# zhangyi-3/UCDIR

Hardware: AMD Instinct MI355X
Metric: restored images/sec at 50-step p_sample_loop, 256x256 SID (higher is better)
Workload: dtype bf16

## Files before the change

### ucdir_amd/csrc/conv_sk.hip.h

```cpp
#pragma once
#include "asmops.hip.h"
#include "conv_halo.hip.h"
#include "akgm_ws.hip.h"

struct ConvSkP {
    const bf16_t* A; long long a_par_stride;
    const bf16_t* B0; const bf16_t* B1; int c0, ld0, ld1;
    int nchunks;
    int nb, H, W, Wp, Hp;
    int ns, Ws, Wpe, HpWpe, npos;
    float inv_per_b, inv_HpWpe, inv_Wpe;
    int ntiles, rowtiles, npar;
    int nhp;
    int nfeat;
    float alpha; int fold; int act;
    const stat_t* stats0; const stat_t* stats1; double inv_count;
    const float* bias; const float* Tb; const float* Tg; int tab_ld;
    const bf16_t* res; int res_ld;
    bf16_t* out; int out_ld;
    stat_t* stats_out;
    int units, ndp;
    float* partial;
    int alt_units; const bf16_t* alt_A; const float* alt_bias; bf16_t* alt_out; int alt_out_ld;
    int mix_wt, mix_nt, mix_nhp, mix_nunits, mix_nndp, mix_q0, mix_srt;
    unsigned long long* dbg;
};

template <int MW, int NW = 8>
struct CvSk {
    static constexpr int NWN = NW / MW;
    static constexpr int NPX = 64 * NWN;
    static constexpr int ROWS = 128 * MW;
    static constexpr int STAGE = 8192 * MW;
    static constexpr int PW = 8 * MW / NW;
    static constexpr bool LDS_TAB = NW == 8;
    static constexpr int OFF_W = 0;
    static constexpr int OFF_TB = 4 * STAGE;
    static constexpr int OFF_TG = OFF_TB + (LDS_TAB ? 9 * ROWS * 4 : 0);
    static constexpr int OFF_MS = OFF_TG + (LDS_TAB ? 9 * ROWS * 4 : 0);
    static constexpr int MAXB = 64;
    static constexpr int OFF_H = OFF_MS + MAXB * 8;
    static constexpr int THREADS = 64 * NW;
    static constexpr int NHW = NW == 4 ? 6 : (MW == 2 ? 4 : 7);
    static constexpr int NHP_MAX = NW * NHW;
    static constexpr int LDS_MAX = NW == 8 ? 160 * 1024 : 80 * 1024;
    __host__ __device__ static constexpr int lds_bytes(int nhp) { return OFF_H + 2 * nhp * 1024; }
    __host__ __device__ static constexpr int part_floats() { return ROWS * NPX; }
};

#ifdef UCDIR_TIMING
#define SK_STAMP() do { if (dbg_on && dbg_n < 120) p.dbg[dbg_off + dbg_n++] = __builtin_amdgcn_s_memtime(); } while (0)
#else
#define SK_STAMP() do {} while (0)
#endif

template <int N>
__device__ __forceinline__ void sk_wait_vm() { asm volatile("s_waitcnt vmcnt(%0)" :: "n"(N) : "memory"); }

struct SkSched {
    int units, ndp, nch, G;
    long long tc;
    __host__ __device__ SkSched(int units_, int ndp_, int nch_, int G_) : units(units_), ndp(ndp_), nch(nch_), G(G_), tc((long long)(units_ - ndp_) * nch_) {}
    __host__ __device__ long long start(int g) const { return tc * g / G; }
};

__device__ __forceinline__ int sk_udiv(int q, int d, float inv_d) {
    int t = (int)((float)q * inv_d);
    t = t * d > q ? t - 1 : t;
    t = (t + 1) * d <= q ? t + 1 : t;
    return t;
}
__device__ __forceinline__ void sk_decode(const ConvSkP& p, int q, int& b, int& yp, int& xs, int& xpm) {
    const int per_b = p.ns * p.HpWpe;
    b = sk_udiv(q, per_b, p.inv_per_b);
    int r = q - b * per_b;
    int strip = 0;
    if (p.ns > 1) { strip = sk_udiv(r, p.HpWpe, p.inv_HpWpe); r -= strip * p.HpWpe; }
    yp = sk_udiv(r, p.Wpe, p.inv_Wpe); xs = r - yp * p.Wpe;
    xpm = strip * p.Ws + xs;
}

__device__ __forceinline__ void lds_read8f_asm(f32x2_t& v, unsigned addr) {
    asm volatile("ds_read_b64 %0, %1" : "=v"(v) : "v"(addr));
}

__device__ __forceinline__ stat_t wave_sum_ll_dpp(stat_t v) {
    auto step = [&](auto ctrl, auto rmask) {
        constexpr int C = decltype(ctrl)::value, RM = decltype(rmask)::value;
// ... 247 lines not shown
        __builtin_amdgcn_sched_barrier(0);
    }
#pragma unroll
    for (int n = 0; n < 2; ++n) {
        const int q = q0 + wn * 64 + n * 32 + l31;
        int b, yp, xs, xp;
        sk_decode(p, q, b, yp, xs, xp);
        const bool valid = q < p.npos && yp >= 1 && yp <= p.H && xs >= 1 && xs <= p.Ws && xp <= p.W;
        const long long opos = ((long long)b * p.Hp + yp) * p.Wp + xp;
#pragma unroll
        for (int f = 0; f < 4; ++f) {
            const int fo = rt * L::ROWS + f * 32 + 16 * hh;
            if (!valid || fo >= p.nfeat) continue;
            float v[16];
#pragma unroll
            for (int g4 = 0; g4 < 4; ++g4) {
                f32x4_t bv = {0.f, 0.f, 0.f, 0.f};
                if (p.alt_bias) bv = *reinterpret_cast<const f32x4_t*>(p.alt_bias + fo + 4 * g4);
#pragma unroll
                for (int e = 0; e < 4; ++e) v[4 * g4 + e] = acc[f][n][4 * g4 + e] + bv[e];
            }
            bf16_t* op = p.alt_out + opos * p.alt_out_ld + fo;
            *reinterpret_cast<uint4*>(op) = pack8_bf16(v);
            *reinterpret_cast<uint4*>(op + 8) = pack8_bf16(v + 8);
        }
    }
}

template <int MW, int NW, int NTAPS, int NF = 4>
__device__ __forceinline__ void conv_sk_body(const ConvSkP& p, unsigned char* smem, const int lid, const int G, const int units_arg, const int ndp_arg,
                                             const int qbase, const int nhp) {
    using L = CvSk<MW, NW>;
    static_assert(NF == 4 || (NF == 2 && MW == 1 && NW == 4), "short units: four waves of 64 x 64");
    constexpr int PWN = L::PW * NF / 4;
    constexpr int RSUB = 4 / NF;
    constexpr int NWN = L::NWN;
    const int tid = threadIdx.x, lane = tid & 63, l31 = lane & 31, hh = lane >> 5;
    const int wave = __builtin_amdgcn_readfirstlane(tid >> 6);
    const int wm = wave / NWN, wn = wave % NWN;
#ifdef UCDIR_TIMING
    const bool dbg_on = p.dbg && (lid == G / 2 + 3 || lid == G - 3) && (lane == 0) && (wave == NW - 1);
    const int dbg_off = lid == G - 3 ? 128 : 0;
    int dbg_n = 0;
#endif
    SK_STAMP();
    const int Wp = p.Wpe, nch = p.nchunks;
    const int HB = nhp * 1024;
    constexpr int NHW = L::NHW;
    constexpr int TA = NTAPS - 3 > 1 ? NTAPS - 3 : 1;
    constexpr int HPER = (NHW + TA - 1) / TA;

    const unsigned a_lane = L::OFF_W + (NF == 4 ? (4 * wm) * 2048 : 0) + lane * 16;
    unsigned bx[NTAPS];
    auto set_bx = [&](int py, int pxp) {
#pragma unroll
        for (int t = 0; t < NTAPS; ++t) {
            int ky, kx;
            if (NTAPS == 9) { ky = t / 3; kx = t - 3 * ky; } else { ky = py + (t >> 1); kx = pxp + (t & 1); }
            const int hp = wn * 64 + l31 + ky * Wp + kx;
            bx[t] = L::OFF_H + (hp << 6) + (((hh ^ (hp >> 2)) & 3) << 4);
        }
    };
    if (NTAPS == 9) set_bx(0, 0);
    const int hpos0 = (lane >> 2) - Wp - 1;
    const unsigned hsw = (unsigned)(((lane & 3) ^ ((lane >> 4) & 3)) << 3);
    auto piece_of = [&](int j) { const int i = j * NW + wave; return i < nhp ? i : nhp - 1; };

    const SkSched sch(units_arg, ndp_arg, nch, G);
    const long long c_beg = sch.start(lid), c_end = sch.start(lid + 1);
    const int ndp_mine = lid < ndp_arg ? (ndp_arg - lid + G - 1) / G : 0;
    long long cpos = c_beg;
    int dpi = 0;
    struct Seg { int unit, cb, ce, par, rt, tile; bool first_sk, ok; };
    auto next_segment = [&]() {
        Seg s; s.ok = true; s.first_sk = false;
        if (dpi < ndp_mine) { s.unit = lid + dpi * G; s.cb = 0; s.ce = nch; ++dpi; }
        else if (cpos < c_end) {
            const long long u = cpos / nch;
            s.unit = ndp_arg + (int)u; s.cb = (int)(cpos - u * nch);
            const long long e = (u + 1) * nch < c_end ? (u + 1) * nch : c_end;
            s.ce = (int)(e - u * nch);
            s.first_sk = cpos == c_beg;
            cpos = e;
        } else { s.ok = false; s.unit = 0; s.cb = 0; s.ce = 0; }
        int u = s.unit;
        const int RT = NF == 4 ? p.rowtiles : p.mix_srt;
        const int per_par = RT * p.ntiles;
        s.par = 0;
        if (p.npar > 1) { s.par = u / per_par; u -= s.par * per_par; }
        s.tile = u / RT; s.rt = u - s.tile * RT;
        return s;
    };

    unsigned hq[NHW];
    int ld_cur = 0;
    const bf16_t* hsrc = nullptr;
    auto halo_chunk = [&](int c) {
        int ch = c * 32;
        const bool first = ch < p.c0;
        const int ld = first ? p.ld0 : p.ld1;
        hsrc = first ? p.B0 + ch : p.B1 + (ch - p.c0);
        if (ld != ld_cur) {
#pragma unroll
            for (int j = 0; j < NHW; ++j) hq[j] = ((((hq[j] >> 1) - hsw) / (unsigned)ld_cur) * (unsigned)ld + hsw) * 2u;
            ld_cur = ld;
        }
    };
    const unsigned char* a_seg = nullptr;
    const unsigned lane16 = (unsigned)lane * 16u;
    int seg_cb = 0;
    auto issue_halo = [&](int j, int buf) {
        dma16_sbase(hsrc, hq[j], (unsigned)(L::OFF_H + piece_of(j) * 1024 + buf * HB));
    };
    auto issue_stage = [&](int k, int slot) {
#pragma unroll
        for (int j = 0; j < PWN; ++j)
            dma16_sbase(a_seg + (long long)k * L::STAGE + j * 1024, lane16, (unsigned)(L::OFF_W + slot * L::STAGE + (wave * PWN + j) * 1024));
    };
    constexpr int NTP = 10;
    auto issue_table = [&](int rt, int i, int buf) {
        const int seg = 2 * i + (lane >> 5);
        const float* src = reinterpret_cast<const float*>(p.A);
        if (seg == 0 || seg > 18) { if (p.bias) src = p.bias + rt * L::ROWS; }
        else if (seg < 10) { if (p.fold) src = p.Tb + (long long)(seg - 1) * p.tab_ld + rt * L::ROWS; }
        else if (p.fold) src = p.Tg + (long long)(seg - 10) * p.tab_ld + rt * L::ROWS;
        __builtin_amdgcn_global_load_lds((const GLOBAL_AS void*)(src + (lane & 31) * 4), (LDS_AS void*)(smem + L::OFF_H + buf * HB + i * 1024), 16, 0, 0);
    };
    int hb0 = 0;
    auto prefetch = [&](const Seg& s) {
        if (NTAPS != 9) set_bx(s.par >> 1, s.par & 1);
        const int q0 = qbase + s.tile * L::NPX;
#pragma unroll
        for (int j = 0; j < NHW; ++j) {
            int q = q0 + hpos0 + 16 * piece_of(j);
            q = q < 0 ? 0 : (q >= p.npos ? (q - p.npos < p.npos ? q - p.npos : 0) : q);
            int b, yp, xs, xp;
            sk_decode(p, q, b, yp, xs, xp);
            xp = xp < p.Wp ? xp : p.Wp - 1;
            hq[j] = (unsigned)((b * p.Hp + yp) * p.Wp + xp);
        }
        ld_cur = s.cb * 32 < p.c0 ? p.ld0 : p.ld1;
#pragma unroll
        for (int j = 0; j < NHW; ++j) hq[j] = (hq[j] * (unsigned)ld_cur + hsw) * 2u;
        halo_chunk(s.cb);
        a_seg = reinterpret_cast<const unsigned char*>(p.A + (long long)s.par * p.a_par_stride + ((long long)(s.rt / RSUB) * nch * NTAPS) * (L::STAGE / 2) +
                                                       (s.rt % RSUB) * (L::STAGE / 2 / RSUB) + (wave * PWN) * 512);
        seg_cb = s.cb;
#pragma unroll
        for (int j = 0; j < NHW; ++j) issue_halo(j, hb0);
#pragma unroll
        for (int k = 0; k < 4; ++k) issue_stage(s.cb * NTAPS + k, k);
    };

    Seg cur = next_segment();
    if (!cur.ok) return;
    int rt_cur = cur.rt;
    prefetch(cur);
    auto sample_range = [&](const Seg& s) {
        const int per_b = p.ns * p.HpWpe;
        const int b0 = sk_udiv(qbase + s.tile * L::NPX, per_b, p.inv_per_b);
        int b1 = sk_udiv(qbase + s.tile * L::NPX + L::NPX - 1, per_b, p.inv_per_b) + 1; b1 = b1 < p.nb ? b1 : p.nb;
        if (b0 < b1) sk_sample_table(p, reinterpret_cast<float*>(smem + L::OFF_MS) + 2 * b0, b0, b1, wave, NW, lane);
    };
    if (L::LDS_TAB) {
        sk_sample_table(p, reinterpret_cast<float*>(smem + L::OFF_MS), 0, p.nb, wave, NW, lane);
        sk_row_table<MW, NW>(p, smem, cur.rt, tid);
    } else sample_range(cur);

#pragma unroll 1
    while (true) {
        const Seg nxt = next_segment();
        const int cb = cur.cb, ce = cur.ce;
        f32x16_t acc[NF][2];
#pragma unroll
        for (int f = 0; f < NF; ++f)
#pragma unroll
            for (int n = 0; n < 2; ++n)
#pragma unroll
                for (int e = 0; e < 16; ++e) acc[f][n][e] = 0.f;

        HC_WAIT(0);
        __builtin_amdgcn_sched_barrier(0);
        asm volatile("s_waitcnt lgkmcnt(0)\n\ts_barrier" ::: "memory");
        SK_STAMP();

        bf16x8_t fa[2][NF], fb[2][2];
        auto reads = [&](auto tc, auto jc, int h, unsigned boff) {
            constexpr int t = decltype(tc)::value, jj = decltype(jc)::value;
            const unsigned aa = a_lane + (unsigned)((h & 3) * L::STAGE);
            lds_read16_asm<0 * 2048 + jj * 1024>(fa[jj][0], aa);
            lds_read16_asm<1 * 2048 + jj * 1024>(fa[jj][1], aa);
            if constexpr (NF == 4) {
                lds_read16_asm<2 * 2048 + jj * 1024>(fa[jj][2], aa);
                lds_read16_asm<3 * 2048 + jj * 1024>(fa[jj][3], aa);
            }
            const unsigned b0 = (bx[t] + boff) ^ (jj << 5);
            lds_read16_asm<0>(fb[jj][0], b0);
            lds_read16_asm<2048>(fb[jj][1], b0);
        };
        __builtin_amdgcn_sched_barrier(0);
        unsigned bcur = hb0 ? (unsigned)HB : 0u;
        reads(std::integral_constant<int, 0>{}, std::integral_constant<int, 0>{}, 0, bcur);
        reads(std::integral_constant<int, 0>{}, std::integral_constant<int, 1>{}, 0, bcur);

        int h = 0;
        const bool want_tab = !L::LDS_TAB && cb == 0 && ce == nch;
#pragma unroll 1
        for (int c = cb; c < ce; ++c) {
            const unsigned bnext = bcur ? 0u : (unsigned)HB;
            const int cn = c + 1 < ce ? c + 1 : c;
            halo_chunk(cn);
            static_for<0, NTAPS>([&](auto tc) {
                constexpr int t = decltype(tc)::value;
                constexpr int tn = (t + 1) % NTAPS;
                constexpr int tm1 = (t + NTAPS - 1) % NTAPS;
                const unsigned boffn = tn == 0 ? bnext : bcur;
                const unsigned aan = a_lane + (unsigned)(((h + 1) & 3) * L::STAGE);
                auto unit = [&](auto jc, auto&& shadow) {
                    constexpr int jj = decltype(jc)::value;
                    const unsigned b0 = (bx[tn] + boffn) ^ (jj << 5);
#define SK_MF(f, n) acc[f][n] = __builtin_amdgcn_mfma_f32_32x32x16_bf16(fa[jj][f], fb[jj][n], acc[f][n], 0, 0, 0); __builtin_amdgcn_sched_barrier(0)
                    if constexpr (NF == 2) {
                        SK_MF(0, 0); shadow(std::integral_constant<int, 0>{}); __builtin_amdgcn_sched_barrier(0);
                        SK_MF(1, 0); lds_read16_asm<0>(fb[jj][0], b0); shadow(std::integral_constant<int, 1>{}); __builtin_amdgcn_sched_barrier(0);
                        SK_MF(0, 1); lds_read16_asm<0 * 2048 + jj * 1024>(fa[jj][0], aan); shadow(std::integral_constant<int, 2>{}); __builtin_amdgcn_sched_barrier(0);
                        SK_MF(1, 1); lds_read16_asm<1 * 2048 + jj * 1024>(fa[jj][1], aan); lds_read16_asm<2048>(fb[jj][1], b0); __builtin_amdgcn_sched_barrier(0);
                    } else {
                    SK_MF(0, 0); shadow(std::integral_constant<int, 0>{}); __builtin_amdgcn_sched_barrier(0);
                    SK_MF(1, 0); shadow(std::integral_constant<int, 1>{}); __builtin_amdgcn_sched_barrier(0);
                    SK_MF(2, 0); shadow(std::integral_constant<int, 2>{}); __builtin_amdgcn_sched_barrier(0);
#ifdef SK_ABL_NOREAD
                    SK_MF(3, 0); SK_MF(0, 1); SK_MF(1, 1); SK_MF(2, 1); SK_MF(3, 1); (void)b0; (void)aan;
#else
                    SK_MF(3, 0); lds_read16_asm<0>(fb[jj][0], b0); __builtin_amdgcn_sched_barrier(0);
                    SK_MF(0, 1); lds_read16_asm<0 * 2048 + jj * 1024>(fa[jj][0], aan); __builtin_amdgcn_sched_barrier(0);
                    SK_MF(1, 1); lds_read16_asm<1 * 2048 + jj * 1024>(fa[jj][1], aan); __builtin_amdgcn_sched_barrier(0);
                    SK_MF(2, 1); lds_read16_asm<2 * 2048 + jj * 1024>(fa[jj][2], aan); __builtin_amdgcn_sched_barrier(0);
                    SK_MF(3, 1); lds_read16_asm<3 * 2048 + jj * 1024>(fa[jj][3], aan); lds_read16_asm<2048>(fb[jj][1], b0); __builtin_amdgcn_sched_barrier(0);
#endif
                    }
#undef SK_MF
                };
#ifndef SK_ABL_NOREAD
                lgkm_wait_asm<NF + 2>();
#endif
                unit(std::integral_constant<int, 0>{}, [&](auto) {});
#ifndef SK_ABL_NOREAD
                lgkm_wait_asm<NF + 2>();
#endif
                {
                    constexpr int j0p = tm1 * HPER < NHW ? tm1 * HPER : NHW, j1p = (tm1 + 1) * HPER < NHW ? (tm1 + 1) * HPER : NHW;
                    constexpr int c1 = tm1 < TA ? j1p - j0p : 0;
#ifndef SK_ABL_NODMA
                    sk_wait_vm<PWN + c1>();
#endif
#ifndef SK_ABL_NOBAR
                    asm volatile("s_barrier" ::: "memory");
#endif
                }
                unit(std::integral_constant<int, 1>{}, [&](auto sc) {
                    constexpr int sidx = decltype(sc)::value;
                    constexpr int j0 = t < TA ? (t * HPER < NHW ? t * HPER : NHW) : 0, j1 = t < TA ? ((t + 1) * HPER < NHW ? (t + 1) * HPER : NHW) : 0;
                    constexpr int nh = j1 - j0;
                    constexpr int total = nh + PWN;
                    static_for<0, total>([&](auto qc) {
                        constexpr int q = decltype(qc)::value;
#ifdef SK_ABL_NODMA
                        constexpr int sh = 99;
#else
                        constexpr int sh = q * 3 / total;
#endif
                        if constexpr (sh == sidx) {
                            if constexpr (q < nh) {
                                constexpr int j = j0 + q;
                                if (want_tab && c + 1 == ce && j * NW + wave < NTP) issue_table(cur.rt / RSUB, j * NW + wave, bnext ? 1 : 0);
                                else issue_halo(j, bnext ? 1 : 0);
                            } else {
                                constexpr int j = q - nh;
                                dma16_sbase(a_seg + (long long)(cb * NTAPS + h + 4) * L::STAGE + j * 1024, lane16, (unsigned)(L::OFF_W + (h & 3) * L::STAGE + (wave * PWN + j) * 1024));
                            }
                        }
                    });
                });
                ++h;
            });
            bcur = bnext;
        }
        asm volatile("s_waitcnt vmcnt(0) lgkmcnt(0)" ::: "memory");
#pragma unroll
        for (int jj = 0; jj < 2; ++jj) {
#pragma unroll
            for (int f = 0; f < NF; ++f) asm volatile("" : "+v"(fa[jj][f]));
            asm volatile("" : "+v"(fb[jj][0]), "+v"(fb[jj][1]));
        }
        __builtin_amdgcn_sched_barrier(0);
        asm volatile("s_barrier" ::: "memory");
        SK_STAMP();
        const bool same_rt = nxt.ok && (nxt.rt == rt_cur || !L::LDS_TAB);
        const unsigned tab_base = (unsigned)L::OFF_H + bcur;
        hb0 = bcur ? 0 : 1;
        if (same_rt) prefetch(nxt);
        __builtin_amdgcn_sched_barrier(0);

        if (NF != 4 || (cb == 0 && ce == nch)) {
            sk_epilogue<MW, NW, L::LDS_TAB ? 1 : 2, true, NF>(p, smem, nullptr, acc, cur.par, cur.rt / RSUB, qbase + cur.tile * L::NPX, wm, wn, lane, tab_base, -1,
                                                             (cur.rt % RSUB) * (32 * NF));
        } else if constexpr (NF == 4) {
            float* pw = p.partial + ((long long)(2 * lid + (cur.first_sk ? 0 : 1))) * L::part_floats() + wave * (128 * 64) + lane * 4;
#pragma unroll
            for (int f = 0; f < 4; ++f)
#pragma unroll
                for (int n = 0; n < 2; ++n)
#pragma unroll
                    for (int g4 = 0; g4 < 4; ++g4)
                        *reinterpret_cast<float4*>(pw + ((f * 2 + n) * 4 + g4) * 256) =
                            make_float4(acc[f][n][4 * g4], acc[f][n][4 * g4 + 1], acc[f][n][4 * g4 + 2], acc[f][n][4 * g4 + 3]);
        }
        SK_STAMP();
        if (!nxt.ok) break;
        if (!same_rt) {
            __syncthreads();
            if (L::LDS_TAB) sk_row_table<MW, NW>(p, smem, nxt.rt, tid);
            rt_cur = nxt.rt;
            prefetch(nxt);
        }
        if (!L::LDS_TAB) { __syncthreads(); sample_range(nxt); }
        cur = nxt;
    }
#ifdef UCDIR_TIMING
    if (dbg_on) p.dbg[dbg_off ? 254 : 255] = dbg_n;
#endif
}

template <int MW, int NW, int NTAPS>
__global__ __launch_bounds__(64 * NW, 2) void conv_sk_kernel(const ConvSkP p) {
    extern __shared__ __attribute__((aligned(16))) unsigned char smem[];
    int lid, G;
    {
        int nblk = gridDim.x, bid = blockIdx.x;
        bool alt = false;
        if (MW == 1 && NW == 4 && p.alt_units) {
// ... 106 lines not shown
```

### ucdir_amd/csrc/engine.hip

```cpp
#include <hip/hip_runtime.h>

#include <algorithm>
#include <cmath>
#include <cstdio>
#include <cstring>
#include <map>
#include <mutex>
#include <set>
#include <array>
#include <atomic>
#include <memory>
#include <string>
#include <vector>

#include "../../include/ucdir_hip.h"
#include "cgemm.hip.h"
#include "conv_halo.hip.h"
#include "akgm_halo.hip.h"
#include "akgm_pre.hip.h"
#include "akgm_ws.hip.h"
#include "akgm_ws32.hip.h"
#include "akgm_ws64.hip.h"
#include "conv_ws.hip.h"
#include "conv_sk.hip.h"
// ... 10 lines not shown
    int rows_pad = 0, Kpad = 0, ntaps = 0, cin = 0, cout = 0, TM = 128; bool fold = false;
    bf16_t* Aup = nullptr; int Kup = 0;
    bf16_t* A10 = nullptr; float* bias_res = nullptr;
    bf16_t* Aws = nullptr;
    bf16_t* Aws128 = nullptr;
    bf16_t* Aqkv = nullptr;
    bf16_t* Atile = nullptr;
    bf16_t* Ask[2] = {nullptr, nullptr}; bf16_t* Ask_up[2] = {nullptr, nullptr};
    long long sk_up_stride[2] = {0, 0};
    bf16_t* Ask1x1 = nullptr;
};
struct AkgmW {
    bf16_t* A = nullptr; float* bias = nullptr; float* Tb = nullptr; float* Tg = nullptr;
    float* Tbb = nullptr;
    bf16_t* Apre = nullptr;
    bf16_t* Aws32 = nullptr;
    bf16_t* Aws64 = nullptr;
    int C = 0, cg = 0, Kpad = 0;
};

static int pick_tm(int cout) { return cout >= 128 ? 128 : 64; }

static ConvW upload_conv(DevPool& pool, const float* w, const float* bias, const float* gamma, const float* beta,
                         int cout, int cin, int ks) {
    ConvW W;
    W.TM = pick_tm(cout);
    PackedConv P = pack_conv(w, bias, gamma, beta, cout, cin, ks, W.TM);
    W.A = pool.upload(P.A); W.bias = pool.upload(P.bias);
    W.fold = gamma != nullptr;
    if (W.fold) { W.Tb = pool.upload(P.Tb); W.Tg = pool.upload(P.Tg); }
    W.rows_pad = P.rows_pad; W.Kpad = P.Kpad; W.ntaps = P.ntaps; W.cin = cin; W.cout = cout;
    if (ks == 3 && cin == 64 && cout == 64 && P.Kpad == 576) W.Aws = pool.upload(pack_conv_ws(P));
    if (ks == 3 && cin % 32 == 0 && P.Kpad == 9 * cin && P.rows_pad % W.TM == 0) W.Atile = pool.upload(pack_conv_tiled(P, W.TM));
    if (ks == 3 && cin % 32 == 0 && P.Kpad == 9 * cin && cout % 128 == 0) {
        W.Ask[0] = pool.upload(pack_conv_sk(P.A, 1, P.rows_pad, P.Kpad, cin, 9, 1));
        if (cout % 256 == 0) W.Ask[1] = pool.upload(pack_conv_sk(P.A, 1, P.rows_pad, P.Kpad, cin, 9, 2));
    }
    if (ks == 1 && cin % 32 == 0 && P.Kpad == cin && cout % 128 == 0 && gamma == nullptr) W.Ask1x1 = pool.upload(pack_conv_sk(P.A, 1, P.rows_pad, P.Kpad, cin, 1, 1));
    if (ks == 1 && cout == 3 * cin && gamma != nullptr && (cin == 256 || cin == 512) && P.Kpad == cin && P.rows_pad >= cout) W.Aqkv = pool.upload(pack_qkv_ws(P, cin));
    return W;
}
static void upload_upconv(DevPool& pool, ConvW& W, const float* w, const float* bias) {
    PackedConv P = pack_upconv(w, bias, W.cout, W.cin, W.TM);
    W.Aup = pool.upload(P.A); W.Kup = P.Kpad;
    for (int mw = 1; mw <= 2; ++mw)
        if (W.cin % 32 == 0 && W.cout % (128 * mw) == 0) {
            std::vector<bf16_t> img = pack_conv_sk(P.A, 4, P.rows_pad, P.Kpad, W.cin, 4, mw);
            W.sk_up_stride[mw - 1] = (long long)((img.size() - (size_t)4 * 4 * mw * 2 * 512) / 4);
            W.Ask_up[mw - 1] = pool.upload(img);
        }
}
static AkgmW upload_akgm(DevPool& pool, const float* wsp, const float* bsp, const float* gamma, const float* beta, int C) {
    PackedAkgm P = pack_akgm(wsp, bsp, gamma, beta, C, 0);
    AkgmW W;
    W.A = pool.upload(P.A); W.bias = pool.upload(P.bias); W.Tb = pool.upload(P.Tb); W.Tg = pool.upload(P.Tg);
    W.C = C; W.cg = P.cg; W.Kpad = P.Kpad;
    {
        std::vector<float> tbb(P.Tb.size());
        const size_t n = P.bias.size();
        for (size_t i = 0; i < tbb.size(); ++i) tbb[i] = P.bias[i % n] + P.Tb[i];
        W.Tbb = pool.upload(tbb);
    }
    if (P.cg == 8 || P.cg == 16) W.Apre = pool.upload(pack_akgm_pre(wsp, gamma, C));
    if (P.cg == 32) W.Aws32 = pool.upload(pack_akgm_ws32(wsp, gamma, C));
    if (P.cg == 64 && C == 512) W.Aws64 = pool.upload(pack_akgm_ws64(wsp, gamma, C));
    return W;
}

struct ProfEntry { int key; double flops, bytes; int dH, dW, dCin, dCout; hipEvent_t e0 = nullptr, e1 = nullptr; };
struct Profiler {
    bool on = false;
    std::vector<ProfEntry> entries;
    std::vector<hipEvent_t> pool; size_t used = 0;
    hipEvent_t get() {
        if (used == pool.size()) { hipEvent_t e; HIPC(hipEventCreate(&e)); pool.push_back(e); }
        return pool[used++];
    }
    ~Profiler() { for (auto e : pool) (void)hipEventDestroy(e); }
};
static Profiler g_prof;
// ... 448 lines not shown
    p.Hi = x0.H; p.Wi = x0.W; p.Wpi = x0.W + 2;
    p.p0 = p.Wp + 1; p.pn = (y.H - 1) * p.Wp + y.W;
    p.ntaps = w.ntaps; p.cg = cin; p.cpt = cin / 8; p.cpt_shift = 0;
    p.nk = w.Kpad / CG_BK;
    p.tiles = (p.pn + CG_TP - 1) / CG_TP;
    p.rowtiles = w.rows_pad / w.TM;
    p.nbatch = y.B;
    p.fold = w.fold ? 1 : 0; p.act = c.act;
    if (w.fold) {
        p.stats0 = x0.stats; p.stats1 = x1 ? x1->stats : nullptr;
        p.inv_count = 1.0 / ((double)cin * x0.H * x0.W);
        p.Tb = w.Tb; p.Tg = w.Tg; p.tab_ld = w.cout;
    }
    p.bias = w.bias;
    if (c.res) { p.res = c.res->p; p.res_bstride = c.res->bstride(); p.res_ld = c.res->C; p.res_coff = 0; }
    p.out = y.p; p.out_bstride = y.bstride(); p.out_ld = y.C; p.nfeat = w.cout;
    if (c.nchw_out) { p.out = c.nchw_out; p.out_nchw = 1; p.crop_h = c.crop_h; p.crop_w = c.crop_w; }
    const bool upph = mode == COLS_UP && w.Aup && x0.C % 64 == 0 && !x1;
    const bool halo = upph || (mode == COLS_S1 && w.ntaps == 9 && x0.C % 64 == 0 && (!x1 || x1->C % 64 == 0));
    if (halo) {
        const int gh = upph ? x0.H : y.H, gw = upph ? x0.W : y.W;
        choose_tile(gh, gw, p.th, p.tw);
        p.tiles_x = (gw + p.tw - 1) / p.tw; p.tiles_y = (gh + p.th - 1) / p.th;
        p.tiles = p.tiles_x * p.tiles_y;
        if (upph) {
            p.up_phase = 1; p.A = w.Aup; p.a_ld = w.Kup; p.a_gstride = (long long)w.rows_pad * w.Kup;
            p.H = x0.H; p.W = x0.W; p.Wp = x0.W + 2;
            p.tiles *= 4;
        }
    }
    if (c.want_stats) {
        p.stats_out = y.stats;
    }
    if (halo && !c.nchw_out && try_conv_sk(w, c, upph, st)) return c.did_res;

    int tm_run = w.TM;
    if (halo && tm_run == 128 && p.nbatch * p.tiles * p.rowtiles < 256) {
        tm_run = 64; p.rowtiles = w.rows_pad / 64;
    }
    bool did_res = false;
    if (halo && !upph && tm_run == 64 && w.TM == 64 && w.A10 && c.res_out && !env().no_fused_res) {
        p.A = w.A10; p.a_ld = 10 * cin; p.res_fused = 1; p.bias2 = w.bias_res;
        p.out2 = c.res_out->p; p.out2_bstride = c.res_out->bstride(); p.out2_ld = c.res_out->C;
        did_res = true;
    }
    const bool dual = did_res;
    if (!env().no_atile && halo && !upph && !did_res && tm_run == w.TM && w.Atile && w.ntaps == 9) p.A_tiled = w.Atile;
    if (halo && !did_res && !p.out_nchw && w.cout % 8 == 0) {
        const int taps = upph ? 4 : 9, tps = 256 / tm_run;
        const int ks = choose_ksplit(p.nbatch * p.tiles * p.rowtiles, cin / HC_BK, (taps + tps - 1) / tps,
                                     (double)y.B * y.H * y.W * w.cout);
        if (ks > 1) { p.ksplit = ks; p.partial = splitk_scratch(); }
    }
    if (halo && !upph && !did_res && c.res_out && c.wres && !env().no_tail_res && !p.out_nchw && c.wres->ntaps == 1 &&
        c.wres->rows_pad >= p.rowtiles * tm_run) {
        p.alt_blocks = p.nbatch * p.tiles * p.rowtiles;
        p.alt_A = c.wres->A; p.alt_a_ld = c.wres->Kpad; p.bias2 = c.wres->bias;
        p.out2 = c.res_out->p; p.out2_bstride = c.res_out->bstride(); p.out2_ld = c.res_out->C;
        did_res = true;
    }
    ConvKind kind = !halo ? ConvKind::CGEMM : tm_run == 128 ? ConvKind::HALO128 : dual ? ConvKind::HALO64_DUAL : ConvKind::HALO64;
    if (!env().no_conv_ws128 && dual && w.Aws128 && cin == 128 && x0.C == 64 && x1 && x1->C == 64 && !c.res && !p.out_nchw && y.H % 8 == 0 && y.W % 16 == 0 &&
        y.C == 64 && (g_persist_grid > 0 || (long long)y.B * (y.H / 8) * (y.W / 16) >= 4LL * num_cus()))
        kind = ConvKind::WS128;
    else if (!env().no_conv_ws && halo && !upph && !did_res && w.Aws && !x1 && !c.res && !p.out_nchw && p.ksplit <= 1 && !p.alt_blocks &&
             y.H % 16 == 0 && y.W % 16 == 0 && x0.C == 64 && y.C == 64 &&
             (g_persist_grid > 0 || (long long)y.B * (y.H / 16) * (y.W / 16) >= 4LL * num_cus()))
// ... 895 lines not shown
    require(name != nullptr, "null argument");
    if (!strcmp(name, "flash")) g_flash = value;
    else if (!strcmp(name, "splitk")) g_splitk = value;
    else if (!strcmp(name, "skmix")) g_skmix = value;
    else if (!strcmp(name, "convsk")) g_convsk = value;
    else if (!strcmp(name, "persist_grid")) g_persist_grid = value;
    else if (!strcmp(name, "reuse_acts")) g_reuse_acts = value < 0 ? -1 : value != 0;
    else throw std::runtime_error(std::string("unknown debug flag ") + name);
    API_END
}

int32_t ucdir_debug_launch_plan(const char* what, int32_t wgs, int32_t nchunks, int32_t steps_per_chunk, double out_elems) {
    if (!what) return -1;
    try {
        if (!strcmp(what, "ksplit")) return choose_ksplit(wgs, nchunks, steps_per_chunk, out_elems);
        if (!strcmp(what, "usplit")) return choose_usplit(wgs);
        if (!strcmp(what, "last_ksplit")) return g_last_ksplit;
        if (!strcmp(what, "tile")) {
            if (wgs < 1 || nchunks < 1) return -1;
            int th = 0, tw = 0;
            choose_tile(wgs, nchunks, th, tw);
            return th * 1000 + tw;
        }
        if (!strcmp(what, "sk_strips")) {
            if (wgs < 1) return -1;
            int ns = 0, Ws = 0, Wpe = 0, nhp = 0;
            bool ok;
            if (nchunks == 14) ok = conv_sk_strips<1, 4>(wgs, ns, Ws, Wpe, nhp);
            else if (nchunks == 28) ok = conv_sk_strips<2, 8>(wgs, ns, Ws, Wpe, nhp);
            else if (nchunks == 18) ok = conv_sk_strips<1, 8>(wgs, ns, Ws, Wpe, nhp);
            else return -1;
            return ok ? ns * 1000 + nhp : 0;
        }
    } catch (...) {}
    return -1;
}

int32_t ucdir_debug_act_plan(const ucdir_config* cfg, int32_t B, int32_t H, int32_t W, int32_t pad_mode, int32_t reuse, int32_t cap,
                             int32_t* rows) {
    try {
        require(cfg && (rows || cap <= 0), "null argument");
        require(cfg->n_mults >= 1 && cfg->n_mults <= UCDIR_MAX_MULTS, "bad n_mults");
        int Hc, Wc;
        plan_compute_size(*cfg, B, H, W, pad_mode, Hc, Wc);
        const std::vector<ActSlot> plan = act_plan(build_layers(*cfg), Hc, Wc, reuse_acts_mode(reuse < 0 ? -1 : reuse != 0, Hc, Wc));
        for (size_t i = 0; i < plan.size() && (int64_t)i < cap; ++i) {
            const ActSlot& s = plan[i];
            const int32_t r[6] = {s.layer, s.which, s.H, s.W, s.C, s.id};
            for (int k = 0; k < 6; ++k) rows[i * 6 + k] = r[k];
        }
        return (int32_t)plan.size();
    }
    catch (const std::exception& e) { fail(e.what()); }
    catch (...) { fail("unknown error"); }
    return -1;
}

int32_t ucdir_profile_enable(int32_t on) {
    API_BEGIN
    g_prof.on = on != 0;
    API_END
}

int32_t ucdir_profile_read(int32_t cap, int32_t* keys, int32_t* launches, double* ms, double* flops, double* bytes,
                           int32_t* nrows, void* stream) {
    API_BEGIN
// ... 413 lines not shown
```

### ucdir_amd/csrc/pack.h

```cpp
#pragma once
#include <cmath>
#include <cstdint>
#include <vector>

#include "common.h"

struct PackedConv {
    std::vector<bf16_t> A;
    std::vector<float> bias;
    std::vector<float> Tb, Tg;
    int rows_pad = 0, Kpad = 0, ntaps = 0, cin = 0, cout = 0, ncls = 0;
};

static inline bool tap_valid(int cls, int tap) {
    const int cy = cls / 3, cx = cls % 3, ky = tap / 3, kx = tap % 3;
    if (cy == 0 && ky == 0) return false;
    if (cy == 2 && ky == 2) return false;
    if (cx == 0 && kx == 0) return false;
    if (cx == 2 && kx == 2) return false;
    return true;
}

static inline PackedConv pack_conv(const float* w, const float* bias, const float* gamma, const float* beta,
                                   int cout, int cin, int ks, int TM) {
// ... 174 lines not shown
            for (int u = 0; u < nsteps; ++u)
                for (int k = 0; k < 16; ++k)
                    for (int lane = 0; lane < 64; ++lane) {
                        const int row = (k % ipt) * 16 + (lane >> 2);
                        int tap = TPS * u + k / ipt; tap = tap < 9 ? tap : 8;
                        const int lc = (lane & 3) ^ ((row >> 2) & 3);
                        const bf16_t* src = &P.A[(size_t)(rt * TM + row) * P.Kpad + (size_t)tap * P.cin + c * 32 + lc * 8];
                        bf16_t* dst = &img[((((size_t)rt * nch + c) * nsteps + u) * 16 + k) * 512 + lane * 8];
                        for (int e = 0; e < 8; ++e) dst[e] = src[e];
                    }
    return img;
}

static inline std::vector<bf16_t> pack_conv_sk(const std::vector<bf16_t>& A, int npar, int rows_pad, int Kld, int cin, int ntaps, int MW) {
    const int ROWS = 128 * MW, nrt = (rows_pad + ROWS - 1) / ROWS, nch = cin / 32, nf = 4 * MW;
    std::vector<bf16_t> img((size_t)npar * nrt * nch * ntaps * nf * 2 * 512 + (size_t)4 * nf * 2 * 512, 0);
    for (int par = 0; par < npar; ++par)
        for (int rt = 0; rt < nrt; ++rt)
            for (int c = 0; c < nch; ++c)
                for (int t = 0; t < ntaps; ++t)
                    for (int f = 0; f < nf; ++f)
                        for (int j = 0; j < 2; ++j)
                            for (int lane = 0; lane < 64; ++lane) {
                                const int rho = lane & 31, hh = lane >> 5;
                                const int row = rt * ROWS + 32 * f + 16 * ((rho >> 2) & 1) + (rho & 3) + 4 * (rho >> 3);
                                if (row >= rows_pad) continue;
                                const bf16_t* src = &A[((size_t)par * rows_pad + row) * Kld + (size_t)t * cin + 32 * c + 16 * j + 8 * hh];
                                bf16_t* dst = &img[(((((((size_t)par * nrt + rt) * nch + c) * ntaps + t) * nf + f) * 2 + j) * 64 + lane) * 8];
                                for (int e = 0; e < 8; ++e) dst[e] = src[e];
                            }
    return img;
}

static inline std::vector<bf16_t> pack_akgm_ws32(const float* wsp, const float* gamma, int C) {
    const int cg = C / 8, nk = 18, nb = C / 32;
    std::vector<bf16_t> img((size_t)nb * 8 * nk * 2 * 32 * 8, 0);
    for (int blk = 0; blk < nb; ++blk)
        for (int w = 0; w < 8; ++w)
            for (int rho = 0; rho < 32; ++rho) {
                const int c4 = 2 * ((rho >> 2) & 1) + (rho >> 4), sm = 4 * ((rho >> 3) & 1) + (rho & 3);
                const int c = 32 * blk + 4 * w + c4, o = 8 * c + sm, g = c / cg;
                for (int j = 0; j < nk; ++j)
                    for (int hk = 0; hk < 2; ++hk)
                        for (int e = 0; e < 8; ++e) {
                            const int tap = j >> 1, ci = 16 * (j & 1) + 8 * hk + e;
                            img[(((((size_t)blk * 8 + w) * nk + j) * 2 + hk) * 32 + rho) * 8 + e] = f2bf(wsp[((size_t)o * cg + ci) * 9 + tap] * gamma[g * cg + ci]);
                        }
            }
    return img;
}

static inline std::vector<bf16_t> pack_akgm_ws64(const float* wsp, const float* gamma, int C) {
    const int cg = C / 8, nk = 36, nh = C / 32;
    std::vector<bf16_t> img((size_t)nh * 8 * nk * 2 * 32 * 8, 0);
    for (int hg = 0; hg < nh; ++hg)
        for (int w = 0; w < 8; ++w)
            for (int rho = 0; rho < 32; ++rho) {
                const int c4 = 2 * ((rho >> 2) & 1) + (rho >> 4), sm = 4 * ((rho >> 3) & 1) + (rho & 3);
                const int c = 32 * hg + 4 * w + c4, o = 8 * c + sm, g = c / cg;
                for (int j = 0; j < nk; ++j)
                    for (int hk = 0; hk < 2; ++hk)
                        for (int e = 0; e < 8; ++e) {
                            const int tap = j >> 2, ci = 16 * (j & 3) + 8 * hk + e;
                            img[(((((size_t)hg * 8 + w) * nk + j) * 2 + hk) * 32 + rho) * 8 + e] = f2bf(wsp[((size_t)o * cg + ci) * 9 + tap] * gamma[g * cg + ci]);
                        }
            }
// ... 56 lines not shown
```

Before: 36.79.

## Switch split-K conv main loop to 16x16x32 MFMA with LDS accumulator relayout

Rewrites the split-K conv inner loop to issue v_mfma_f32_16x16x32_bf16 on 16-row weight fragments instead of 32x32x16, with a new weight packing (pack_conv_sk16) and a new halo swizzle. After the K loop the 16x16 accumulators are staged through LDS in the weight ring to rebuild the 32x32 accumulator layout the existing epilogue expects. This adds a round trip through LDS, barriers and s_nop padding per segment in exchange for a different read/MFMA interleave and fewer halo bank conflicts. The sk path also becomes usable for non-halo COLS_S1 3x3 convs when forced, and a host-side bank-conflict estimator is added.

```diff
diff --git a/ucdir_amd/csrc/conv_sk.hip.h b/ucdir_amd/csrc/conv_sk.hip.h
--- a/ucdir_amd/csrc/conv_sk.hip.h
+++ b/ucdir_amd/csrc/conv_sk.hip.h
@@ -54,6 +54,33 @@
 #define SK_STAMP() do {} while (0)
 #endif
 
+__host__ __device__ constexpr unsigned sk_halo_chunk(unsigned c, unsigned hp) { return (c ^ ((hp >> 1) & 2u)) & 3u; }
+inline int sk_halo_read_cycles(int Wpe, int ky, int kx, int wn) {
+    static const int group_of[16] = {0, 0, 0, 0, 1, 1, 1, 1, 1, 1, 1, 1, 0, 0, 0, 0};
+    int cycles = 0;
+    for (int grp = 0; grp < 4; ++grp) {
+        unsigned addr_of_bank[64][16]; int n_of_bank[64] = {0};
+        for (int lane = 0; lane < 64; ++lane) {
+            const int g = (lane >> 5) * 2 + ((lane & 16) ? 1 - group_of[lane & 15] : group_of[lane & 15]);
+            if (g != grp) continue;
+            const unsigned hp = (unsigned)(wn * 64 + (lane & 15) + ky * Wpe + kx);
+            const unsigned addr = (hp << 6) + (sk_halo_chunk((unsigned)(lane >> 4), hp) << 4);
+            for (int d = 0; d < 4; ++d) {
+                const int bank = (int)((addr / 4 + d) & 63);
+                bool seen = false;
+                for (int i = 0; i < n_of_bank[bank]; ++i) seen = seen || addr_of_bank[bank][i] == addr;
+                if (!seen) addr_of_bank[bank][n_of_bank[bank]++] = addr;
+            }
+        }
+        int worst = 1;
+        for (int b = 0; b < 64; ++b) worst = n_of_bank[b] > worst ? n_of_bank[b] : worst;
+        cycles += worst;
+    }
+    return cycles;
+}
+
+__device__ __forceinline__ int sk_opaque(int v) { asm volatile("" : "+v"(v)); return v; }
+
 template <int N>
 __device__ __forceinline__ void sk_wait_vm() { asm volatile("s_waitcnt vmcnt(%0)" :: "n"(N) : "memory"); }
 
@@ -367,8 +394,10 @@
                                              const int qbase, const int nhp) {
     using L = CvSk<MW, NW>;
     static_assert(NF == 4 || (NF == 2 && MW == 1 && NW == 4), "short units: four waves of 64 x 64");
+    static_assert(NW * 4096 <= 4 * L::STAGE, "the layout conversion's 4 KB per wave come out of the weight ring");
     constexpr int PWN = L::PW * NF / 4;
     constexpr int RSUB = 4 / NF;
+    constexpr int NA = 2 * NF, HA = NF;
     constexpr int NWN = L::NWN;
     const int tid = threadIdx.x, lane = tid & 63, l31 = lane & 31, hh = lane >> 5;
     const int wave = __builtin_amdgcn_readfirstlane(tid >> 6);
@@ -392,13 +421,13 @@
         for (int t = 0; t < NTAPS; ++t) {
             int ky, kx;
             if (NTAPS == 9) { ky = t / 3; kx = t - 3 * ky; } else { ky = py + (t >> 1); kx = pxp + (t & 1); }
-            const int hp = wn * 64 + l31 + ky * Wp + kx;
-            bx[t] = L::OFF_H + (hp << 6) + (((hh ^ (hp >> 2)) & 3) << 4);
+            const int hp = wn * 64 + (lane & 15) + ky * Wp + kx;
+            bx[t] = L::OFF_H + (hp << 6) + (sk_halo_chunk((unsigned)(lane >> 4), (unsigned)hp) << 4);
         }
     };
     if (NTAPS == 9) set_bx(0, 0);
     const int hpos0 = (lane >> 2) - Wp - 1;
-    const unsigned hsw = (unsigned)(((lane & 3) ^ ((lane >> 4) & 3)) << 3);
+    const unsigned hsw = sk_halo_chunk((unsigned)(lane & 3), (unsigned)(lane >> 2)) << 3;
     auto piece_of = [&](int j) { const int i = j * NW + wave; return i < nhp ? i : nhp - 1; };
 
     const SkSched sch(units_arg, ndp_arg, nch, G);
@@ -454,12 +483,12 @@
     };
     constexpr int NTP = 10;
     auto issue_table = [&](int rt, int i, int buf) {
-        const int seg = 2 * i + (lane >> 5);
+        const int ln = sk_opaque(lane), seg = 2 * i + (ln >> 5);
         const float* src = reinterpret_cast<const float*>(p.A);
         if (seg == 0 || seg > 18) { if (p.bias) src = p.bias + rt * L::ROWS; }
         else if (seg < 10) { if (p.fold) src = p.Tb + (long long)(seg - 1) * p.tab_ld + rt * L::ROWS; }
         else if (p.fold) src = p.Tg + (long long)(seg - 10) * p.tab_ld + rt * L::ROWS;
-        __builtin_amdgcn_global_load_lds((const GLOBAL_AS void*)(src + (lane & 31) * 4), (LDS_AS void*)(smem + L::OFF_H + buf * HB + i * 1024), 16, 0, 0);
+        __builtin_amdgcn_global_load_lds((const GLOBAL_AS void*)(src + (ln & 31) * 4), (LDS_AS void*)(smem + L::OFF_H + buf * HB + i * 1024), 16, 0, 0);
     };
     int hb0 = 0;
     auto prefetch = [&](const Seg& s) {
@@ -495,7 +524,7 @@
         const int per_b = p.ns * p.HpWpe;
         const int b0 = sk_udiv(qbase + s.tile * L::NPX, per_b, p.inv_per_b);
         int b1 = sk_udiv(qbase + s.tile * L::NPX + L::NPX - 1, per_b, p.inv_per_b) + 1; b1 = b1 < p.nb ? b1 : p.nb;
-        if (b0 < b1) sk_sample_table(p, reinterpret_cast<float*>(smem + L::OFF_MS) + 2 * b0, b0, b1, wave, NW, lane);
+        if (b0 < b1) sk_sample_table(p, reinterpret_cast<float*>(smem + L::OFF_MS) + 2 * b0, b0, b1, wave, NW, sk_opaque(lane));
     };
     if (L::LDS_TAB) {
         sk_sample_table(p, reinterpret_cast<float*>(smem + L::OFF_MS), 0, p.nb, wave, NW, lane);
@@ -506,37 +535,34 @@
     while (true) {
         const Seg nxt = next_segment();
         const int cb = cur.cb, ce = cur.ce;
-        f32x16_t acc[NF][2];
-#pragma unroll
-        for (int f = 0; f < NF; ++f)
-#pragma unroll
-            for (int n = 0; n < 2; ++n)
-#pragma unroll
-                for (int e = 0; e < 16; ++e) acc[f][n][e] = 0.f;
+        f32x4_t c16[NA][4];
+#pragma unroll
+        for (int r = 0; r < NA; ++r)
+#pragma unroll
+            for (int n = 0; n < 4; ++n) c16[r][n] = f32x4_t{0.f, 0.f, 0.f, 0.f};
 
         HC_WAIT(0);
         __builtin_amdgcn_sched_barrier(0);
         asm volatile("s_waitcnt lgkmcnt(0)\n\ts_barrier" ::: "memory");
         SK_STAMP();
 
-        bf16x8_t fa[2][NF], fb[2][2];
-        auto reads = [&](auto tc, auto jc, int h, unsigned boff) {
-            constexpr int t = decltype(tc)::value, jj = decltype(jc)::value;
-            const unsigned aa = a_lane + (unsigned)((h & 3) * L::STAGE);
-            lds_read16_asm<0 * 2048 + jj * 1024>(fa[jj][0], aa);
-            lds_read16_asm<1 * 2048 + jj * 1024>(fa[jj][1], aa);
-            if constexpr (NF == 4) {
-                lds_read16_asm<2 * 2048 + jj * 1024>(fa[jj][2], aa);
-                lds_read16_asm<3 * 2048 + jj * 1024>(fa[jj][3], aa);
-            }
-            const unsigned b0 = (bx[t] + boff) ^ (jj << 5);
-            lds_read16_asm<0>(fb[jj][0], b0);
-            lds_read16_asm<2048>(fb[jj][1], b0);
-        };
+        bf16x8_t fa[NA], fb[4];
+#ifdef SK_ABL_NOREAD
+        auto rd_a = [&](auto, unsigned) {};
+        auto rd_b = [&](auto, unsigned) {};
+#else
+        auto rd_a = [&](auto rc, unsigned aa) { constexpr int r = decltype(rc)::value; lds_read16_asm<r * 1024>(fa[r], aa); };
+        auto rd_b = [&](auto nc, unsigned b0) { constexpr int n = decltype(nc)::value; lds_read16_asm<n * 1024>(fb[n], b0); };
+#endif
         __builtin_amdgcn_sched_barrier(0);
         unsigned bcur = hb0 ? (unsigned)HB : 0u;
-        reads(std::integral_constant<int, 0>{}, std::integral_constant<int, 0>{}, 0, bcur);
-        reads(std::integral_constant<int, 0>{}, std::integral_constant<int, 1>{}, 0, bcur);
+        {
+            const unsigned b0 = bx[0] + bcur;
+            static_for<0, HA>([&](auto rc) { rd_a(rc, a_lane); });
+            static_for<0, 3>([&](auto nc) { rd_b(nc, b0); });
+            static_for<HA, NA>([&](auto rc) { rd_a(rc, a_lane); });
+            rd_b(std::integral_constant<int, 3>{}, b0);
+        }
 
         int h = 0;
         const bool want_tab = !L::LDS_TAB && cb == 0 && ce == nch;
@@ -551,38 +577,25 @@
                 constexpr int tm1 = (t + NTAPS - 1) % NTAPS;
                 const unsigned boffn = tn == 0 ? bnext : bcur;
                 const unsigned aan = a_lane + (unsigned)(((h + 1) & 3) * L::STAGE);
-                auto unit = [&](auto jc, auto&& shadow) {
-                    constexpr int jj = decltype(jc)::value;
-                    const unsigned b0 = (bx[tn] + boffn) ^ (jj << 5);
-#define SK_MF(f, n) acc[f][n] = __builtin_amdgcn_mfma_f32_32x32x16_bf16(fa[jj][f], fb[jj][n], acc[f][n], 0, 0, 0); __builtin_amdgcn_sched_barrier(0)
-                    if constexpr (NF == 2) {
-                        SK_MF(0, 0); shadow(std::integral_constant<int, 0>{}); __builtin_amdgcn_sched_barrier(0);
-                        SK_MF(1, 0); lds_read16_asm<0>(fb[jj][0], b0); shadow(std::integral_constant<int, 1>{}); __builtin_amdgcn_sched_barrier(0);
-                        SK_MF(0, 1); lds_read16_asm<0 * 2048 + jj * 1024>(fa[jj][0], aan); shadow(std::integral_constant<int, 2>{}); __builtin_amdgcn_sched_barrier(0);
-                        SK_MF(1, 1); lds_read16_asm<1 * 2048 + jj * 1024>(fa[jj][1], aan); lds_read16_asm<2048>(fb[jj][1], b0); __builtin_amdgcn_sched_barrier(0);
-                    } else {
-                    SK_MF(0, 0); shadow(std::integral_constant<int, 0>{}); __builtin_amdgcn_sched_barrier(0);
-                    SK_MF(1, 0); shadow(std::integral_constant<int, 1>{}); __builtin_amdgcn_sched_barrier(0);
-                    SK_MF(2, 0); shadow(std::integral_constant<int, 2>{}); __builtin_amdgcn_sched_barrier(0);
-#ifdef SK_ABL_NOREAD
-                    SK_MF(3, 0); SK_MF(0, 1); SK_MF(1, 1); SK_MF(2, 1); SK_MF(3, 1); (void)b0; (void)aan;
-#else
-                    SK_MF(3, 0); lds_read16_asm<0>(fb[jj][0], b0); __builtin_amdgcn_sched_barrier(0);
-                    SK_MF(0, 1); lds_read16_asm<0 * 2048 + jj * 1024>(fa[jj][0], aan); __builtin_amdgcn_sched_barrier(0);
-                    SK_MF(1, 1); lds_read16_asm<1 * 2048 + jj * 1024>(fa[jj][1], aan); __builtin_amdgcn_sched_barrier(0);
-                    SK_MF(2, 1); lds_read16_asm<2 * 2048 + jj * 1024>(fa[jj][2], aan); __builtin_amdgcn_sched_barrier(0);
-                    SK_MF(3, 1); lds_read16_asm<3 * 2048 + jj * 1024>(fa[jj][3], aan); lds_read16_asm<2048>(fb[jj][1], b0); __builtin_amdgcn_sched_barrier(0);
+                const unsigned b0n = bx[tn] + boffn;
+                auto half = [&](auto hc, auto&& shadow) {
+                    constexpr int hf = decltype(hc)::value;
+                    static_for<0, 4 * HA>([&](auto mc) {
+                        constexpr int m = decltype(mc)::value, n = m / HA, r = hf * HA + m % HA;
+                        if constexpr (hf == 0 && m % HA == 0) {
+#ifndef SK_ABL_NOREAD
+                            lgkm_wait_asm<n == 3 ? 0 : HA + 3 - n>();
 #endif
-                    }
-#undef SK_MF
+                        }
+                        asm volatile("v_mfma_f32_16x16x32_bf16 %0, %1, %2, %0" : "+v"(c16[r][n]) : "v"(fa[r]), "v"(fb[n]));
+                        __builtin_amdgcn_sched_barrier(0);
+                        if constexpr (hf == 1 && m < 3) shadow(mc);
+                        if constexpr (n == 3) rd_a(std::integral_constant<int, r>{}, aan);
+                        if constexpr (hf == 1 && m % HA == HA - 1) rd_b(std::integral_constant<int, n>{}, b0n);
+                        __builtin_amdgcn_sched_barrier(0);
+                    });
                 };
-#ifndef SK_ABL_NOREAD
-                lgkm_wait_asm<NF + 2>();
-#endif
-                unit(std::integral_constant<int, 0>{}, [&](auto) {});
-#ifndef SK_ABL_NOREAD
-                lgkm_wait_asm<NF + 2>();
-#endif
+                half(std::integral_constant<int, 0>{}, [&](auto) {});
                 {
                     constexpr int j0p = tm1 * HPER < NHW ? tm1 * HPER : NHW, j1p = (tm1 + 1) * HPER < NHW ? (tm1 + 1) * HPER : NHW;
                     constexpr int c1 = tm1 < TA ? j1p - j0p : 0;
@@ -593,7 +606,7 @@
                     asm volatile("s_barrier" ::: "memory");
 #endif
                 }
-                unit(std::integral_constant<int, 1>{}, [&](auto sc) {
+                half(std::integral_constant<int, 1>{}, [&](auto sc) {
                     constexpr int sidx = decltype(sc)::value;
                     constexpr int j0 = t < TA ? (t * HPER < NHW ? t * HPER : NHW) : 0, j1 = t < TA ? ((t + 1) * HPER < NHW ? (t + 1) * HPER : NHW) : 0;
                     constexpr int nh = j1 - j0;
@@ -621,27 +634,52 @@
             });
             bcur = bnext;
         }
-        asm volatile("s_waitcnt vmcnt(0) lgkmcnt(0)" ::: "memory");
-#pragma unroll
-        for (int jj = 0; jj < 2; ++jj) {
-#pragma unroll
-            for (int f = 0; f < NF; ++f) asm volatile("" : "+v"(fa[jj][f]));
-            asm volatile("" : "+v"(fb[jj][0]), "+v"(fb[jj][1]));
-        }
+        asm volatile("s_waitcnt vmcnt(0) lgkmcnt(0)\n\ts_nop 15\n\ts_nop 15" ::: "memory");
+#pragma unroll
+        for (int r = 0; r < NA; ++r) asm volatile("" : "+v"(fa[r]));
+#pragma unroll
+        for (int n = 0; n < 4; ++n) asm volatile("" : "+v"(fb[n]));
         __builtin_amdgcn_sched_barrier(0);
         asm volatile("s_barrier" ::: "memory");
         SK_STAMP();
+        f32x16_t acc[NF][2];
+        {
+            const int ln = sk_opaque(lane);
+            const int l15 = ln & 15, p31 = ln & 31, ph = ln >> 5;
+            const unsigned sbase = (unsigned)(L::OFF_W + wave * 4096);
+            const unsigned w0 = sbase + (unsigned)(l15 * 128 + ((((ln >> 4) ^ (l15 & 7) ^ (l15 >> 3)) & 7) << 4));
+            const unsigned w1 = w0 ^ 64u;
+            const unsigned r0 = sbase + (unsigned)(p31 * 128 + ((((ph << 2) ^ (p31 & 7) ^ ((p31 >> 3) & 1)) & 7) << 4));
+            const unsigned r1 = r0 ^ 16u, r2 = r0 ^ 32u, r3 = r0 ^ 48u;
+#pragma unroll
+            for (int f = 0; f < NF; ++f)
+#pragma unroll
+                for (int n = 0; n < 2; ++n) {
+                    asm volatile("ds_write_b128 %0, %1" :: "v"(w0), "v"(c16[2 * f][2 * n]) : "memory");
+                    asm volatile("ds_write_b128 %0, %1 offset:2048" :: "v"(w0), "v"(c16[2 * f][2 * n + 1]) : "memory");
+                    asm volatile("ds_write_b128 %0, %1" :: "v"(w1), "v"(c16[2 * f + 1][2 * n]) : "memory");
+                    asm volatile("ds_write_b128 %0, %1 offset:2048" :: "v"(w1), "v"(c16[2 * f + 1][2 * n + 1]) : "memory");
+                    asm volatile("s_waitcnt lgkmcnt(0)" ::: "memory");
+                    f32x4_t t0, t1, t2, t3;
+                    lds_read16f_asm<0>(t0, r0); lds_read16f_asm<0>(t1, r1); lds_read16f_asm<0>(t2, r2); lds_read16f_asm<0>(t3, r3);
+                    asm volatile("s_waitcnt lgkmcnt(0)" ::: "memory");
+                    asm volatile("" : "+v"(t0), "+v"(t1), "+v"(t2), "+v"(t3));
+                    __builtin_amdgcn_sched_barrier(0);
+                    const f32x8_t lo = __builtin_shufflevector(t0, t1, 0, 1, 2, 3, 4, 5, 6, 7), hi = __builtin_shufflevector(t2, t3, 0, 1, 2, 3, 4, 5, 6, 7);
+                    acc[f][n] = __builtin_shufflevector(lo, hi, 0, 1, 2, 3, 4, 5, 6, 7, 8, 9, 10, 11, 12, 13, 14, 15);
+                }
+        }
         const bool same_rt = nxt.ok && (nxt.rt == rt_cur || !L::LDS_TAB);
         const unsigned tab_base = (unsigned)L::OFF_H + bcur;
         hb0 = bcur ? 0 : 1;
-        if (same_rt) prefetch(nxt);
+        if (same_rt) { asm volatile("s_barrier" ::: "memory"); prefetch(nxt); }
         __builtin_amdgcn_sched_barrier(0);
 
         if (NF != 4 || (cb == 0 && ce == nch)) {
             sk_epilogue<MW, NW, L::LDS_TAB ? 1 : 2, true, NF>(p, smem, nullptr, acc, cur.par, cur.rt / RSUB, qbase + cur.tile * L::NPX, wm, wn, lane, tab_base, -1,
                                                              (cur.rt % RSUB) * (32 * NF));
         } else if constexpr (NF == 4) {
-            float* pw = p.partial + ((long long)(2 * lid + (cur.first_sk ? 0 : 1))) * L::part_floats() + wave * (128 * 64) + lane * 4;
+            float* pw = p.partial + ((long long)(2 * lid + (cur.first_sk ? 0 : 1))) * L::part_floats() + wave * (128 * 64) + sk_opaque(lane) * 4;
 #pragma unroll
             for (int f = 0; f < 4; ++f)
 #pragma unroll
diff --git a/ucdir_amd/csrc/engine.hip b/ucdir_amd/csrc/engine.hip
--- a/ucdir_amd/csrc/engine.hip
+++ b/ucdir_amd/csrc/engine.hip
@@ -66,11 +66,11 @@
     W.rows_pad = P.rows_pad; W.Kpad = P.Kpad; W.ntaps = P.ntaps; W.cin = cin; W.cout = cout;
     if (ks == 3 && cin == 64 && cout == 64 && P.Kpad == 576) W.Aws = pool.upload(pack_conv_ws(P));
     if (ks == 3 && cin % 32 == 0 && P.Kpad == 9 * cin && P.rows_pad % W.TM == 0) W.Atile = pool.upload(pack_conv_tiled(P, W.TM));
-    if (ks == 3 && cin % 32 == 0 && P.Kpad == 9 * cin && cout % 128 == 0) {
-        W.Ask[0] = pool.upload(pack_conv_sk(P.A, 1, P.rows_pad, P.Kpad, cin, 9, 1));
-        if (cout % 256 == 0) W.Ask[1] = pool.upload(pack_conv_sk(P.A, 1, P.rows_pad, P.Kpad, cin, 9, 2));
-    }
-    if (ks == 1 && cin % 32 == 0 && P.Kpad == cin && cout % 128 == 0 && gamma == nullptr) W.Ask1x1 = pool.upload(pack_conv_sk(P.A, 1, P.rows_pad, P.Kpad, cin, 1, 1));
+    if (ks == 3 && cin % 32 == 0 && cout % 128 == 0) {
+        W.Ask[0] = pool.upload(pack_conv_sk16(P.A, 1, P.rows_pad, P.Kpad, cin, 9, 1));
+        if (cout % 256 == 0) W.Ask[1] = pool.upload(pack_conv_sk16(P.A, 1, P.rows_pad, P.Kpad, cin, 9, 2));
+    }
+    if (ks == 1 && cin % 32 == 0 && cout % 128 == 0 && gamma == nullptr) W.Ask1x1 = pool.upload(pack_conv_sk(P.A, 1, P.rows_pad, P.Kpad, cin, 1, 1));
     if (ks == 1 && cout == 3 * cin && gamma != nullptr && (cin == 256 || cin == 512) && P.Kpad == cin && P.rows_pad >= cout) W.Aqkv = pool.upload(pack_qkv_ws(P, cin));
     return W;
 }
@@ -79,7 +79,7 @@
     W.Aup = pool.upload(P.A); W.Kup = P.Kpad;
     for (int mw = 1; mw <= 2; ++mw)
         if (W.cin % 32 == 0 && W.cout % (128 * mw) == 0) {
-            std::vector<bf16_t> img = pack_conv_sk(P.A, 4, P.rows_pad, P.Kpad, W.cin, 4, mw);
+            std::vector<bf16_t> img = pack_conv_sk16(P.A, 4, P.rows_pad, P.Kpad, W.cin, 4, mw);
             W.sk_up_stride[mw - 1] = (long long)((img.size() - (size_t)4 * 4 * mw * 2 * 512) / 4);
             W.Ask_up[mw - 1] = pool.upload(img);
         }
@@ -594,7 +594,8 @@
     if (c.want_stats) {
         p.stats_out = y.stats;
     }
-    if (halo && !c.nchw_out && try_conv_sk(w, c, upph, st)) return c.did_res;
+    const bool sk_forced = g_convsk.load() > 0 && mode == COLS_S1 && w.ntaps == 9;
+    if ((halo || sk_forced) && !c.nchw_out && try_conv_sk(w, c, upph, st)) return c.did_res;
 
     int tm_run = w.TM;
     if (halo && tm_run == 128 && p.nbatch * p.tiles * p.rowtiles < 256) {
@@ -1556,6 +1557,10 @@
             else return -1;
             return ok ? ns * 1000 + nhp : 0;
         }
+        if (!strcmp(what, "sk_halo_cycles")) {
+            if (wgs < 1 || nchunks < 0 || nchunks > 8 || steps_per_chunk < 0 || steps_per_chunk > 7) return -1;
+            return sk_halo_read_cycles(wgs, nchunks / 3, nchunks % 3, steps_per_chunk);
+        }
     } catch (...) {}
     return -1;
 }
diff --git a/ucdir_amd/csrc/pack.h b/ucdir_amd/csrc/pack.h
--- a/ucdir_amd/csrc/pack.h
+++ b/ucdir_amd/csrc/pack.h
@@ -230,6 +230,24 @@
     return img;
 }
 
+static inline std::vector<bf16_t> pack_conv_sk16(const std::vector<bf16_t>& A, int npar, int rows_pad, int Kld, int cin, int ntaps, int MW) {
+    const int ROWS = 128 * MW, nrt = (rows_pad + ROWS - 1) / ROWS, nch = cin / 32, nf = 8 * MW;
+    std::vector<bf16_t> img((size_t)npar * nrt * nch * ntaps * nf * 512 + (size_t)4 * nf * 512, 0);
+    for (int par = 0; par < npar; ++par)
+        for (int rt = 0; rt < nrt; ++rt)
+            for (int c = 0; c < nch; ++c)
+                for (int t = 0; t < ntaps; ++t)
+                    for (int R = 0; R < nf; ++R)
+                        for (int lane = 0; lane < 64; ++lane) {
+                            const int row = rt * ROWS + 16 * R + (lane & 15), g = lane >> 4;
+                            if (row >= rows_pad) continue;
+                            const bf16_t* src = &A[((size_t)par * rows_pad + row) * Kld + (size_t)t * cin + 32 * c + 8 * g];
+                            bf16_t* dst = &img[((((((size_t)par * nrt + rt) * nch + c) * ntaps + t) * nf + R) * 64 + lane) * 8];
+                            for (int e = 0; e < 8; ++e) dst[e] = src[e];
+                        }
+    return img;
+}
+
 static inline std::vector<bf16_t> pack_akgm_ws32(const float* wsp, const float* gamma, int C) {
     const int cg = C / 8, nk = 18, nb = C / 32;
     std::vector<bf16_t> img((size_t)nb * 8 * nk * 2 * 32 * 8, 0);
```

Result: faster. 37.29 (median of 6 runs) (+1.4%).
